# RashmikaDushan/MocapV2

Hardware: AMD Instinct MI355X
Metric: frames/sec (6-cam 1080p) (higher is better)
Workload: dtype u8+int64+f64; 1 GPU; 6-camera 1920x1080 synthetic IR frames, 8 markers (BASELINE.json configs[1]); cameras=6, width=1920, height=1080, markers=8, distortion=mild, frames_resident_in_hbm=True, batches_in_flight=3, resident_batches=3, status_ok=True, input=gray frames, parallelism=single launch, time-major

## Files before the change

include/mocap_hip.h:

```cpp
#ifndef MOCAP_HIP_H
#define MOCAP_HIP_H

#include <stddef.h>
#include <stdint.h>

#ifdef __cplusplus
extern "C" {
#endif

#define MOCAP_ABI_VERSION 7
#define MOCAP_API __attribute__((visibility("default")))

enum {
    MOCAP_OK = 0,
    MOCAP_E_INVALID = -1,
    MOCAP_E_HIP = -2,
    MOCAP_E_UNSUPPORTED = -3,
    MOCAP_E_STATE = -4
};

enum {
    MOCAP_BLOB_E_CANDIDATES = -2,
    MOCAP_BLOB_E_CONTOURS = -3,
    MOCAP_BLOB_E_STEPS = -4,
// ... 128 lines not shown
MOCAP_API int mocap_intrinsics_linearize(mocap_ctx_t ctx, int n_cams, const int32_t* view_offset_host,
                                         const int32_t* point_offset_host, const double* obj_xy_dev, const double* img_uv_dev,
                                         const double* kd_dev, const double* view_poses_dev, double lambda, double* cost_dev,
                                         double* gradient_dev, double* S_dev, double* rhs_dev, int32_t* status_dev, void* stream);

#define MOCAP_COMM_ID_BYTES 128
MOCAP_API int mocap_comm_unique_id(void* id_out );
MOCAP_API int mocap_comm_available(void);
MOCAP_API int mocap_comm_init(mocap_ctx_t ctx, const void* id , int rank, int world);
MOCAP_API int mocap_comm_share(mocap_ctx_t dst, mocap_ctx_t src);
MOCAP_API int mocap_comm_destroy(mocap_ctx_t ctx);
MOCAP_API int mocap_allgather_centroids(mocap_ctx_t ctx, const int32_t* local_records_dev, int32_t* gathered_dev,
                                        long ints_per_rank, void* stream);

MOCAP_API int mocap_tile_stats(mocap_ctx_t ctx, uint64_t* tiles, uint64_t* skipped);
MOCAP_API int mocap_profile_enable(mocap_ctx_t ctx, int on);
MOCAP_API int mocap_profile_read(mocap_ctx_t ctx, double ms[5], int launches[5]);

#ifdef __cplusplus
}
#endif
#endif
```

mocapv2_amd/_abi.py:

```python
import ctypes as C
import os

_HERE = os.path.dirname(os.path.abspath(__file__))
LIB_PATH = os.path.join(_HERE, "libmocap_hip.so")
ABI_VERSION = 7
COMM_ID_BYTES = 128


class MocapError(RuntimeError):
    def __init__(self, code, msg):
        super().__init__(f"libmocap_hip error {code}: {msg}")
        self.code = code


class BlobParams(C.Structure):
    _fields_ = [("ksize", C.c_int32), ("median", C.c_int32), ("thresh", C.c_double), ("min_area", C.c_double),
                ("min_circ", C.c_double)]


class UndistortInfo(C.Structure):
    _fields_ = [("identity", C.c_int32), ("compact_table", C.c_int32), ("early_out_provable", C.c_int32),
                ("max_source_weight", C.c_int32), ("sparse_path", C.c_int32)]


# ... 33 lines not shown
    "mocap_ba_residuals": [_vp, _dp, _i, _vp, _vp, _i, _i, C.POINTER(C.c_float), _ip, _vp],
    "mocap_fundamental_ransac": [_vp, _i, _vp, _vp, _ip, _vp, _i, _d, _i, _vp, _vp, _vp, _vp, _vp, _vp],
    "mocap_rig_bundle_adjust": [_vp, _i, _i, _i, _vp, _vp, _vp, _vp, _vp, _i, _d, _d, _vp, _vp, _vp],
    "mocap_rig_linearize": [_vp, _i, _i, _i, _vp, _vp, _vp, _vp, _vp, _d, _vp, _vp, _vp, _vp, _vp, _vp],
    "mocap_intrinsics_calibrate": [_vp, _i, _ip, _ip, _vp, _vp, _ip, _i, _i, _d, _d, _vp, _vp, _vp, _vp, _vp, _vp],
    "mocap_intrinsics_linearize": [_vp, _i, _ip, _ip, _vp, _vp, _vp, _vp, _d, _vp, _vp, _vp, _vp, _vp, _vp],
    "mocap_triangulate_batch": [_vp, _vp, _vp, _i, _i, _i, _vp, _vp, _vp],
    "mocap_reproject_batch": [_vp, _vp, _vp, _vp, _i, _i, _i, _vp, _vp, _vp],
    "mocap_comm_unique_id": [_vp],
    "mocap_comm_available": [],
    "mocap_comm_init": [_vp, _vp, _i, _i],
    "mocap_comm_share": [_vp, _vp],
    "mocap_comm_destroy": [_vp],
    "mocap_allgather_centroids": [_vp, _vp, _vp, _l, _vp],
    "mocap_tile_stats": [_vp, C.POINTER(C.c_uint64), C.POINTER(C.c_uint64)],
    "mocap_profile_enable": [_vp, _i],
    "mocap_profile_read": [_vp, _dp, _ip],
}

_lib = None


def load():
    global _lib
    if _lib is not None:
        return _lib
    if not os.path.exists(LIB_PATH):
        raise RuntimeError(f"{LIB_PATH} is missing: build it with `make -C mocapv2_amd/csrc` "
                           "(hipcc --offload-arch=gfx950); there is no CPU fallback")
    try:
# ... 19 lines not shown
```

mocapv2_amd/csrc/abi.hip:

```cpp
#include <hip/hip_runtime.h>
#include <stdint.h>
#include <stdio.h>
#include <stdarg.h>
#include <stdlib.h>
#include <string.h>
#include <math.h>
#include <string>
#include <vector>
#include <mutex>
#include <memory>
#include <dlfcn.h>
#include "../../include/mocap_hip.h"
#include "kernels.h"

using namespace mocap;

static_assert(sizeof(mocap_contour) == sizeof(ContourRec), "debug record layout");

static thread_local std::string g_err;

static int fail(int code, const char* fmt, ...)
{
    char buf[512];
    va_list ap;
// ... 54 lines not shown
        (void)hipSetDevice(device);
        if (last) { if (have_last) (void)hipEventSynchronize(last); (void)hipEventDestroy(last); }
        if (comm && destroy_comm) (void)destroy_comm(comm);
    }
};

struct Tuning {
    int rows = 68;
    int general_filter = 0;
    int skip_dark = 1;
    int dense_boxes = 0;
    int remap_pipeline = 1;
    int cluster = 1;
    int wide_quads_remap = 34, wide_quads_identity = 34;
    int wide_bands = 1;
    int wide_fork = 0;
    int box_prio = 0, scan_prio = 0, contour_prio = 0, corr_prio = 0;
    int box_stage_bytes = BOX_SCAP;
    int box_blocks_per_cu = 0;
    int box_timing = 0, contour_timing = 0, follow_timing = 0;
    int scan_wide = 1;
    int rows_staged = 0;
    int wide_blocks_per_cu = 3;
    int rows_stage_dw = -1;
    int scan_serial = 1;
    int scan_hotmap = 1;
    int scan_blocks_per_cu = 0;
    int scan_slices = 1;
    int excess_base = -1;
    int base_sel = 1;
    int probe_debug = 0;
    int contour_boxes = 1;
    int contours_split = 1;
    int contour_defer = 1;
    int mark_blocks_per_cu = 0;
    int contour_blocks_per_cu = 0;
    int corr_threads = 256;
    int corr_step_groups = 0;
};
struct TuneName { const char* name; int Tuning::*field; int lo, hi; };
static const TuneName kTuneNames[] = {
    {"rows", &Tuning::rows, 16, 68}, {"general_filter", &Tuning::general_filter, 0, 1}, {"skip_dark", &Tuning::skip_dark, 0, 1},
    {"dense_boxes", &Tuning::dense_boxes, 0, 1}, {"remap_pipeline", &Tuning::remap_pipeline, 0, 1}, {"cluster", &Tuning::cluster, 0, 1},
    {"wide_quads_remap", &Tuning::wide_quads_remap, 0, 100000}, {"wide_quads_identity", &Tuning::wide_quads_identity, 0, 100000},
    {"wide_bands", &Tuning::wide_bands, 1, 4}, {"wide_fork", &Tuning::wide_fork, 0, 1},
    {"box_prio", &Tuning::box_prio, 0, 1}, {"scan_prio", &Tuning::scan_prio, 0, 3}, {"contour_prio", &Tuning::contour_prio, 0, 3},
    {"corr_prio", &Tuning::corr_prio, 0, 3}, {"box_stage_bytes", &Tuning::box_stage_bytes, 0, BOX_SCAP},
    {"box_blocks_per_cu", &Tuning::box_blocks_per_cu, 0, 32}, {"box_timing", &Tuning::box_timing, 0, 1},
    {"contour_timing", &Tuning::contour_timing, 0, 1}, {"follow_timing", &Tuning::follow_timing, 0, 2}, {"scan_wide", &Tuning::scan_wide, 0, 1}, {"scan_hotmap", &Tuning::scan_hotmap, 0, 2}, {"scan_serial", &Tuning::scan_serial, 0, 1}, {"rows_staged", &Tuning::rows_staged, 0, 1}, {"wide_blocks_per_cu", &Tuning::wide_blocks_per_cu, 1, 8}, {"rows_stage_dw", &Tuning::rows_stage_dw, -1, 1 << 20}, {"scan_blocks_per_cu", &Tuning::scan_blocks_per_cu, 0, 64}, {"scan_slices", &Tuning::scan_slices, 1, 64}, {"excess_base", &Tuning::excess_base, -1, 254},
    {"base_sel", &Tuning::base_sel, 0, 1}, {"probe_debug", &Tuning::probe_debug, 0, 1}, {"contour_boxes", &Tuning::contour_boxes, 0, 1},
    {"contours_split", &Tuning::contours_split, 0, 1}, {"contour_blocks_per_cu", &Tuning::contour_blocks_per_cu, 0, 16}, {"mark_blocks_per_cu", &Tuning::mark_blocks_per_cu, 0, 16}, {"contour_defer", &Tuning::contour_defer, 0, 2}, {"corr_threads", &Tuning::corr_threads, 64, 256},
    {"corr_step_groups", &Tuning::corr_step_groups, 0, 0x7fffffff},
};
static bool tune_set(Tuning& t, const char* name, int v)
{
    for (const TuneName& n : kTuneNames)
        if (!strcmp(n.name, name)) {
            t.*(n.field) = v < n.lo ? n.lo : (v > n.hi ? n.hi : v);
            return true;
        }
// ... 377 lines not shown
    if (c->cells && c->last_images > 0) {
        HIP_TRY(hipDeviceSynchronize());
        Tiling t = tiling(c);
        size_t per = cells_per_image(c), n = per * (size_t)c->last_images;
        std::vector<uint32_t> w(n);
        HIP_TRY(hipMemcpy(w.data(), c->cells, sizeof(uint32_t) * n, hipMemcpyDeviceToHost));
        int valid_chunks = (c->H + t.rows - 1) / t.rows;
        total = (uint64_t)c->last_images * valid_chunks * t.n_strips;
        for (size_t i = 0; i < n; i++) full += w[i] >> 31;
    }
    if (tiles) *tiles = total;
    if (skipped) *skipped = total - full;
    return MOCAP_OK;
}

static int check_frames(mocap_ctx* c, const void* frames, int n_images, int cam_mod, int slot_base, size_t image_stride, int pitch)
{
    if (!c || !frames) return fail(MOCAP_E_INVALID, "null argument");
    if (n_images < 1) return fail(MOCAP_E_INVALID, "n_images = %d", n_images);
    if (cam_mod < 1 || slot_base < 0 || slot_base + cam_mod > c->n_slots)
        return fail(MOCAP_E_INVALID, "slots %d..%d not in 0..%d", slot_base, slot_base + cam_mod - 1, c->n_slots - 1);
    if (pitch < c->W) return fail(MOCAP_E_INVALID, "pitch %d < width %d", pitch, c->W);
    if (n_images > 1 && image_stride < (size_t)pitch * (c->H - 1) + c->W) return fail(MOCAP_E_INVALID, "image_stride too small");
    for (int s = slot_base; s < slot_base + cam_mod; s++)
        if (c->slot_state[s] == 0) return fail(MOCAP_E_STATE, "mocap_set_undistort was not called for slot %d", s);
    return 0;
}


static int excess_base(int thr_mul, int sel)
// ... 154 lines not shown
    a.srcbox = c->srcbox ? c->srcbox + (size_t)bt.slot_base * source_cells(c) : nullptr;
    a.remap_bits = p.remap_bits;
    a.cam_mod = bt.cam_mod; a.n_images = bt.n_images; a.n_steps = (bt.n_images + bt.cam_mod - 1) / bt.cam_mod;
    a.thr_mul = sb.thr_mul;
    a.rows_per_chunk = tl.rows; a.n_strips = tl.n_strips; a.n_chunks = tl.n_cgroups * 4;
    const size_t tr_words = c->mask_images * cells_per_image(c) * 4;
    a.tile_rows = c->tile_rows + (c->tile_rows_flip ? tr_words : 0);
    a.tile_rows_next = c->tile_rows + (c->tile_rows_flip ? 0 : tr_words);
    a.n_clear = c->tile_rows_hold[c->tile_rows_flip ^ 1];
    a.cluster = c->tune.cluster;
    a.cur_box = bt.own_mask ? c->cur_box : c->cur_box_ext;
    a.items = c->items; a.n_items = c->n_items; a.cap_items = (uint32_t)c->items.n;
    a.dense = sb.allow < 0;
    a.wide_tiles = c->wide_tiles; a.cap_wide = (uint32_t)c->wide_tiles.n; a.wide_quads_remap = c->tune.wide_quads_remap; a.wide_quads_identity = c->tune.wide_quads_identity;
    a.wide_bands = c->tune.wide_bands;
    if (c->W < 4 || p.direct) a.wide_tiles = nullptr;
    a.bayer = p.direct ? p.bl : BayerArgs{};
    a.stage_bytes = c->tune.box_stage_bytes;
    a.prio = c->tune.box_prio;
    a.ext_mask = bt.own_mask ? 0 : 1;
    return a;
}

static BrightArgs bright_args(const mocap_ctx* c, const Batch& bt, const FilterPath& p, const ScanBounds& sb, uint32_t* tile_rows, bool scan_zeroes)
{
    const Tiling tl = tiling(c);
    uint64_t ncx64 = (uint64_t)((c->W + 7) / 8);
    const uint64_t ncells = ncx64 * (uint64_t)((c->H + 7) / 8);
    int wide = (c->W % 16 == 0) && (bt.pitch % 16 == 0) && (bt.image_stride % 16 == 0) && (((uintptr_t)p.frames & 15) == 0) && ncx64 >= 4;
    if (wide && ncells * (ncx64 / 2) >= (1ull << 32)) wide = 0;
// ... 79 lines not shown

static int report_box_timing(mocap_ctx* c, const uint64_t* timing, hipStream_t s)
{
    std::vector<uint64_t> t((size_t)6 * c->box_grid);
    HIP_TRY(hipStreamSynchronize(s));
    HIP_TRY(hipMemcpy(t.data(), timing, sizeof(uint64_t) * t.size(), hipMemcpyDeviceToHost));
    double sum[6] = {0, 0, 0, 0, 0, 0}, mx = 0;
    for (int b = 0; b < c->box_grid; b++) {
        double tot = 0;
        for (int i = 0; i < 6; i++) { sum[i] += (double)t[6 * b + i]; if (i < 5) tot += (double)t[6 * b + i]; }
        mx = tot > mx ? tot : mx;
    }
    const double n = sum[5] > 0 ? sum[5] : 1;
    uint32_t cnt[16];
    HIP_TRY(hipMemcpy(cnt, c->n_items, sizeof(cnt), hipMemcpyDeviceToHost));
    fprintf(stderr, "[box] list: %u items, %u wide-tile entries\n", cnt[0], cnt[8]);
    fprintf(stderr, "[box] items %.0f (%.1f per wave) | cycles per item: header+wait %.0f, stage %.0f, patch %.0f, threshold %.0f, majority+next %.0f | busiest wave %.0f cycles\n",
            sum[5], sum[5] / c->box_grid, sum[0] / n, sum[1] / n, sum[2] / n, sum[3] / n, sum[4] / n, mx);
    return 0;
}

static int filter_boxes(mocap_ctx* c, const Batch& bt, const FilterPath& p, BoxArgs& a)
{
    const hipStream_t s = bt.s;
    Buf<uint64_t> timing;
    if (c->tune.box_timing) {
        TRY(timing.reserve((size_t)6 * c->box_grid));
        HIP_TRY(hipMemsetAsync(timing, 0, sizeof(uint64_t) * 6 * c->box_grid, s));
    }
    a.timing = timing;
    EvPair ev; bool on;
// ... 166 lines not shown
    EvPair p; bool on;
    prof_begin(c, 1, s, p, on);
    launch_contours(a, s);
    prof_end(c, 1, s, p, on);
    HIP_TRY(hipGetLastError());
    if (follow_dbg) TRY(report_follow_timing(follow_dbg, a.follow_grid, s));
    if (timing) TRY(report_contour_timing(timing, n_images, s));
    return 0;
}

static int grow_mask_group(mocap_ctx* c, size_t n_images)
{
    const size_t tiles = n_images * cells_per_image(c);
    TRY(c->mask.reserve(n_images * mask_image_words(c->H, c->wpr), true));
    TRY(c->cells.reserve(tiles, true));
    std::vector<uint32_t> init(tiles * 4);
    for (size_t i = 0; i < init.size(); i += 2) { init[i] = 0xffffffffu; init[i + 1] = 0u; }
    TRY(c->tile_rows.reserve(2 * init.size()));
    HIP_TRY(hipMemcpy(c->tile_rows, init.data(), sizeof(uint32_t) * init.size(), hipMemcpyHostToDevice));
    HIP_TRY(hipMemcpy(c->tile_rows + init.size(), init.data(), sizeof(uint32_t) * init.size(), hipMemcpyHostToDevice));
    const int hw0 = hot_map_words(c->H, c->W, 0), hw1 = hot_map_words(c->H, c->W, 1);
    TRY(c->hotmap.reserve(n_images * (hw0 > hw1 ? hw0 : hw1), true));
    for (size_t i = 0; i < init.size(); i++) init[i] = 1u;
    TRY(c->cur_box.reserve(init.size()));
    HIP_TRY(hipMemcpy(c->cur_box, init.data(), sizeof(uint32_t) * init.size(), hipMemcpyHostToDevice));
    const size_t cap = tiles * BOX_MAX_PARTS;
    if (cap > 0xffffffffull) return fail(MOCAP_E_UNSUPPORTED, "batch too large for the work list");
    TRY(c->items.reserve(cap));
    return c->wide_tiles.reserve(4 * tiles);
}
static int ensure_mask(mocap_ctx* c, int n_images)
{
// ... 602 lines not shown
```

mocapv2_amd/csrc/blob_boxes.hip:

```cpp
#include <hip/hip_runtime.h>
#include <stdint.h>
#include <type_traits>
#include "kernels.h"
#include "bayer.h"

namespace mocap {

namespace {

__device__ __forceinline__ uint32_t from_prev(uint32_t v)
{
    return (uint32_t)__builtin_amdgcn_update_dpp(0, (int)v, 0x138 , 0xf, 0xf, true);
}
__device__ __forceinline__ uint32_t from_next(uint32_t v)
{
    return (uint32_t)__builtin_amdgcn_update_dpp(0, (int)v, 0x130 , 0xf, 0xf, true);
}
__device__ __forceinline__ uint32_t dot4(uint32_t a, uint32_t sel, uint32_t acc) { return __builtin_amdgcn_udot4(a, sel, acc, false); }
__device__ __forceinline__ int uni(int v) { return __builtin_amdgcn_readfirstlane(v); }
__device__ __forceinline__ int imin(int a, int b) { return a < b ? a : b; }
__device__ __forceinline__ int imax(int a, int b) { return a > b ? a : b; }
__device__ __forceinline__ int taps5(int v, int n)
{
    int lo = v - 2 < 0 ? 0 : v - 2, hi = v + 2 > n - 1 ? n - 1 : v + 2;
// ... 76 lines not shown
__device__ __forceinline__ void choose_split(int nb, int h, int& nx, int& ny)
{
    int best = 0x7fffffff;
    nx = 1; ny = 1;
    for (int cx = 1; cx <= 4; cx++) {
        const int pb = (nb + cx - 1) / cx, Q = 2 * pb + 2;
        if (Q > 64) continue;
        const int rpw = 64 / Q, mr = BOX_HCAP / Q - 8;
        if (mr < 1) continue;
        const int cy = (h + mr - 1) / mr;
        if (cx * cy > BOX_MAX_PARTS) continue;
        const int ph = (h + cy - 1) / cy;
        const int cost = cx * cy * ((ph + 8 + rpw - 1) / rpw + 8);
        if (cost < best) { best = cost; nx = cx; ny = cy; }
    }
}

__global__ __launch_bounds__(256) void settle_tiles_kernel(BoxArgs a)
{
    const int lane = threadIdx.x & 63;
    if (a.zero8 && blockIdx.x == 0 && threadIdx.x < 8) a.zero8[threadIdx.x] = 0u;
    const int tiles = a.n_chunks * a.n_strips;
    const int n_all = a.n_clear > a.n_images ? a.n_clear : a.n_images;
    const int steps_all = (n_all + a.cam_mod - 1) / a.cam_mod;
    const long long total = (long long)tiles * a.cam_mod * steps_all;
    const long long i = (long long)blockIdx.x * 256 + threadIdx.x;
    int image = 0, chunk = 0, strip = 0;
    bool valid = i < total;
    if (valid) {
        const int t = (int)(i % steps_all);
        const long long rest = i / steps_all;
        const int slot = (int)(rest % a.cam_mod), tile = (int)(rest / a.cam_mod);
        image = t * a.cam_mod + slot;
        chunk = tile / a.n_strips; strip = tile - chunk * a.n_strips;
        valid = chunk * a.rows_per_chunk < a.H;
    }
    const size_t idx = ((size_t)image * a.n_chunks + chunk) * a.n_strips + strip;
    if (valid && !a.dense && image < n_all) {
        const uint4 nxt = *(const uint4*)(a.tile_rows_next + 4 * idx);
        if (nxt.x <= nxt.y) *(uint4*)(a.tile_rows_next + 4 * idx) = make_uint4(0xffffffffu, 0u, 0xffffffffu, 0u);
    }
    valid = valid && image < a.n_images;
    const int tile_r0 = chunk * a.rows_per_chunk, tile_r1 = imin(tile_r0 + a.rows_per_chunk, a.H) - 1;
    const int tile_x0 = 240 * strip, tile_x1 = imin(tile_x0 + 239, a.W - 1);
    int bx0 = 0, bx1 = a.W - 1, by0 = 0, by1 = a.H - 1;
    bool marked = valid;
    uint4 raw = make_uint4(0xffffffffu, 0u, 0xffffffffu, 0u);
    if (valid && !a.dense) {
        raw = *(const uint4*)(a.tile_rows + 4 * idx);
        marked = raw.x <= raw.y;
        if (marked) { by0 = (int)raw.x; by1 = (int)raw.y; bx0 = (int)raw.z; bx1 = (int)raw.w; }
    }
    int ox0 = imax(bx0, tile_x0) & ~7, ox1 = imin(imin(bx1, tile_x1) | 7, tile_x1);
    int oy0 = imax(by0, tile_r0), oy1 = imin(by1, tile_r1);
    if (marked && (ox0 > ox1 || oy0 > oy1)) marked = false;
    if (!marked) { ox0 = 1; ox1 = 0; oy0 = 1; oy1 = 0; }
    int nx = 0, ny = 0, nb = 0, h = 0;
    bool wide = false;
    int ix0 = ox0, ix1 = ox1, iy0 = oy0, iy1 = oy1;
    int ux0 = bx0, ux1 = bx1, uy0 = by0, uy1 = by1;
    bool emits = marked;
    if (marked && !a.dense && a.cluster) {
        const int c0 = chunk & ~1, s0 = strip & ~1;
        int n_marked = 0, first = -1, X0 = 0x7fffffff, X1 = -1, Y0 = 0x7fffffff, Y1 = -1;
        for (int k = 0; k < 4; k++) {
            const int cy = c0 + (k >> 1), sx = s0 + (k & 1);
            if (cy >= a.n_chunks || sx >= a.n_strips || cy * a.rows_per_chunk >= a.H) continue;
            const uint4 o = *(const uint4*)(a.tile_rows + 4 * (((size_t)image * a.n_chunks + cy) * a.n_strips + sx));
            if (o.x > o.y) continue;
            if (first < 0) first = k;
            n_marked++;
            Y0 = imin(Y0, (int)o.x); Y1 = imax(Y1, (int)o.y); X0 = imin(X0, (int)o.z); X1 = imax(X1, (int)o.w);
        }
        if (n_marked >= 2) {
            const int bx_lo = 240 * s0, bx_hi = imin(240 * (s0 + 2) - 1, a.W - 1), by_lo = c0 * a.rows_per_chunk, by_hi = imin((c0 + 2) * a.rows_per_chunk, a.H) - 1;
            const int ex0 = imax(X0, bx_lo) & ~7, ex1 = imin(X1 | 7, bx_hi), ey0 = imax(Y0, by_lo), ey1 = imin(Y1, by_hi);
            if (((ex1 - ex0 + 8) >> 3) <= 13 && ey1 - ey0 + 1 <= 100) {
                emits = first == ((chunk - c0) * 2 + (strip - s0));
                ix0 = ex0; ix1 = ex1; iy0 = ey0; iy1 = ey1;
                ux0 = X0; ux1 = X1; uy0 = Y0; uy1 = Y1;
            }
        }
    }
    if (marked) {
        nb = (ix1 - ix0 + 8) >> 3; h = iy1 - iy0 + 1;
        choose_split(nb, h, nx, ny);
        const int slot_ = image % a.cam_mod;
        const int limit = ((a.remap_bits >> slot_) & 1ull) ? a.wide_quads_remap : a.wide_quads_identity;
        wide = emits && ix0 == ox0 && ix1 == ox1 && iy0 == oy0 && iy1 == oy1 && a.wide_tiles != nullptr && 2 * nb + 2 * nx >= limit;
        if (wide) { ox0 = tile_x0; ox1 = tile_x1; ix0 = ox0; ix1 = ox1; }
    }
    const uint32_t nout_x = (uint32_t)ox0 | ((uint32_t)ox1 << 16), nout_y = (uint32_t)oy0 | ((uint32_t)oy1 << 16);

    bool need_clear = false;
    uint32_t pout_x = 1u, pout_y = 1u;
    if (valid) {
        uint4* cb = (uint4*)(a.cur_box + 4 * idx);
        if (!a.ext_mask) {
            const uint4 prev = *cb;
            pout_x = prev.x; pout_y = prev.y;
            const int px0 = (int)(prev.x & 0xffffu), px1 = (int)(prev.x >> 16), py0 = (int)(prev.y & 0xffffu), py1 = (int)(prev.y >> 16);
            if (px0 <= px1) need_clear = !(marked && ox0 <= px0 && px1 <= ox1 && oy0 <= py0 && py1 <= oy1);
            if (prev.x != nout_x || prev.y != nout_y || marked)
                *cb = make_uint4(nout_x, nout_y, (uint32_t)bx0 | ((uint32_t)bx1 << 16), (uint32_t)by0 | ((uint32_t)by1 << 16));
            if (a.cells[idx] != 0u) a.cells[idx] = 0u;
        } else {
            *cb = make_uint4(nout_x, nout_y, (uint32_t)bx0 | ((uint32_t)bx1 << 16), (uint32_t)by0 | ((uint32_t)by1 << 16));
            a.cells[idx] = 0u;
        }
    }
    for (uint64_t todo = __ballot(need_clear); todo; todo &= todo - 1) {
        const int src = __ffsll((long long)todo) - 1;
        const uint32_t cx = (uint32_t)__builtin_amdgcn_readlane((int)pout_x, src), cy = (uint32_t)__builtin_amdgcn_readlane((int)pout_y, src);
        const int cimage = __builtin_amdgcn_readlane(image, src);
        const int x0 = (int)(cx & 0xffffu), x1 = (int)(cx >> 16), y0 = (int)(cy & 0xffffu), y1 = (int)(cy >> 16);
        uint8_t* m = (uint8_t*)(a.mask + (size_t)cimage * mask_image_words(a.H, a.words_per_row));
        const int b0 = x0 >> 3, nr = y1 - y0 + 1, n = nr * ((x1 >> 3) - b0 + 1);
// ... 6 lines not shown
    if (uint64_t wb = __ballot(wide)) {
        const int nbands = a.wide_bands;
        uint32_t base_w = 0;
        if (lane == 0) base_w = atomicAdd(a.n_items + 8, (uint32_t)(__popcll(wb) * nbands));
        base_w = (uint32_t)__builtin_amdgcn_readfirstlane((int)base_w);
        const uint32_t ow = base_w + (uint32_t)(__popcll(wb & ((1ull << lane) - 1ull)) * nbands);
        if (wide) {
            const int hb = (oy1 - oy0 + nbands) / nbands;
            for (int b = 0; b < nbands; b++) {
                const int y0 = oy0 + b * hb, y1 = imin(y0 + hb - 1, oy1);
                if (ow + b < a.cap_wide)
                    a.wide_tiles[ow + b] = make_uint4((uint32_t)image, (uint32_t)(chunk * a.n_strips + strip), (uint32_t)y0, (uint32_t)(y0 <= y1 ? y1 : y0 - 1));
            }
        }
    }
    const int cnt = (wide || !emits) ? 0 : nx * ny;
    int incl = cnt;
#pragma unroll
    for (int d = 1; d < 64; d <<= 1) {
        const int o = __shfl_up(incl, d);
        if (lane >= d) incl += o;
    }
    const int wave_total = __builtin_amdgcn_readlane(incl, 63);
    if (wave_total == 0) return;
    uint32_t base = 0;
    if (lane == 0) base = atomicAdd(a.n_items, (uint32_t)wave_total);
    base = (uint32_t)__builtin_amdgcn_readfirstlane((int)base);
    uint32_t o = base + (uint32_t)(incl - cnt);
    if (cnt) {
        const int pb = (nb + nx - 1) / nx, ph = (h + ny - 1) / ny;
        for (int jy = 0; jy < ny; jy++)
            for (int jx = 0; jx < nx; jx++, o++) {
                const int x0 = ix0 + 8 * pb * jx, x1 = imin(x0 + 8 * pb - 1, ix1);
                const int y0 = iy0 + ph * jy, y1 = imin(y0 + ph - 1, iy1);
                if (o >= a.cap_items) continue;
                uint4 it;
                it.x = (uint32_t)image;
                it.y = (uint32_t)(chunk * a.n_strips + strip);
                it.z = (uint32_t)x0 | ((uint32_t)x1 << 16);
                it.w = (uint32_t)y0 | ((uint32_t)y1 << 16);
                if (x0 > x1 || y0 > y1) it.z = 1u;
                ((uint4*)a.items)[2 * o] = it;
                ((uint4*)a.items)[2 * o + 1] = make_uint4((uint32_t)ux0 | ((uint32_t)ux1 << 16), (uint32_t)uy0 | ((uint32_t)uy1 << 16), 0u, 0u);
            }
// ... 537 lines not shown
```

mocapv2_amd/csrc/blob_filter.hip:

```cpp
#include <hip/hip_runtime.h>
#include <stdint.h>
#include <type_traits>
#include "kernels.h"
#include "scan_mark.h"

namespace mocap {

__device__ __forceinline__ uint32_t lane_from_prev(uint32_t v)
{
    return (uint32_t)__builtin_amdgcn_update_dpp(0, (int)v, 0x138 , 0xf, 0xf, true);
}
__device__ __forceinline__ uint32_t lane_from_next(uint32_t v)
{
    return (uint32_t)__builtin_amdgcn_update_dpp(0, (int)v, 0x130 , 0xf, 0xf, true);
}
__device__ __forceinline__ uint32_t dot4(uint32_t a, uint32_t sel, uint32_t acc)
{
    return __builtin_amdgcn_udot4(a, sel, acc, false);
}

__device__ __forceinline__ uint32_t load_u32(const uint8_t* p)
{
    uint32_t v;
    __builtin_memcpy(&v, p, 4);
// ... 172 lines not shown
            const int c = 8 * cx, cc = c < a.W - 8 ? c : a.W - 8;
            sh[u] = (uint32_t)(8 * (c - cc));
#pragma unroll
            for (int j = 0; j < 8; j++) {
                int r = 8 * cr[u] + j;
                r = r < a.H ? r : a.H - 1;
                __builtin_memcpy(&v[u][j], img + ((uint32_t)r * (uint32_t)a.pitch + (uint32_t)cc), 8);
            }
        }
    }
    const int slot = image % a.cam_mod;
    const uint2* __restrict__ reach = a.reach + (size_t)slot * n;
    const uint8_t* __restrict__ cflags = a.cflags + (size_t)slot * n;
    uint32_t* __restrict__ rows = a.tile_rows + (size_t)image * a.n_chunks * a.n_strips * 4;
    const uint32_t base4 = (uint32_t)a.base * 0x01010101u, c8 = 8u * (uint32_t)a.base;
    uint32_t level[2] = {0u, 0u};
#pragma unroll
    for (int u = 0; u < 2; u++) {
        uint32_t acc = 0;
#pragma unroll
        for (int j = 0; j < 8; j++) {
            if (WIDE) {
                const uint32_t e2 = excess2_row(v[u][j].x, v[u][j].y, base4, c8);
                if (FULL || 8 * cr[u] + j < a.H) acc += e2;
            } else {
                uint64_t vv = (((uint64_t)v[u][j].y << 32) | v[u][j].x) >> sh[u];
                const uint32_t e2 = excess2_row((uint32_t)vv, (uint32_t)(vv >> 32), base4, c8);
                if (8 * cr[u] + j < a.H) acc += e2;
            }
        }
        if (MAP) level[u] = in_range[u] ? hot_level(a, acc) : 0u;
        else mark_hot_cell(a, reach, cflags, rows, ci[u], acc);
        if (a.probe && (image & 15) == 0) {
            const uint32_t alt4 = (uint32_t)a.base_alt * 0x01010101u, alt8 = 8u * (uint32_t)a.base_alt;
            uint32_t acc2 = 0;
#pragma unroll
            for (int j = 0; j < 8; j++) {
                const uint64_t vv = WIDE ? (((uint64_t)v[u][j].y << 32) | v[u][j].x) : ((((uint64_t)v[u][j].y << 32) | v[u][j].x) >> sh[u]);
                const uint32_t e2 = excess2_row((uint32_t)vv, (uint32_t)(vv >> 32), alt4, alt8);
                if (FULL || 8 * cr[u] + j < a.H) acc2 += e2;
            }
            const int n_cur = __popcll(__ballot((int)acc > a.hot)), n_alt = __popcll(__ballot((int)acc2 > a.hot_alt));
            if ((threadIdx.x & 63) == 0) {
                atomicAdd(&a.probe[PROBE_STRIDE * (bx & 127)], (uint32_t)n_cur);
                atomicAdd(&a.probe[PROBE_STRIDE * (bx & 127) + 1], (uint32_t)n_alt);
            }
        }
    }
    if (MAP) {
        const int lane = threadIdx.x & 63;
        uint32_t* __restrict__ hm = a.hotmap + (size_t)image * a.hot_words;
        if (WIDE) {
            uint32_t w = (level[0] | (level[1] << 2)) << (4 * (lane & 7));
            w |= (uint32_t)__builtin_amdgcn_update_dpp(0, (int)w, 0xB1 , 0xf, 0xf, true);
            w |= (uint32_t)__builtin_amdgcn_update_dpp(0, (int)w, 0x4E , 0xf, 0xf, true);
            w |= (uint32_t)__builtin_amdgcn_update_dpp(0, (int)w, 0x141 , 0xf, 0xf, true);
            if ((lane & 7) == 0 && w != 0u) hm[(bx * 256 + (int)threadIdx.x) >> 3] = w;
        } else {
#pragma unroll
            for (int u = 0; u < 2; u++) {
                uint32_t w = level[u] << (2 * (lane & 15));
                w |= (uint32_t)__builtin_amdgcn_update_dpp(0, (int)w, 0xB1, 0xf, 0xf, true);
// ... 15 lines not shown
    const int n_cells = ((a.W + 7) >> 3) * ((a.H + 7) >> 3);
    for (long long piece = (long long)blockIdx.x * 4 + wv; piece < (long long)wpi * a.n_images; piece += (long long)gridDim.x * 4) {
    const int image = (int)(piece / wpi), wave_word0 = (int)(piece - (long long)image * wpi) * 256;
    uint32_t* __restrict__ hm = a.hotmap + (size_t)image * a.hot_words;
    uint32_t wk[4];
#pragma unroll
    for (int k = 0; k < 4; k++) {
        const int wi = wave_word0 + 64 * k + lane;
        wk[k] = wi < a.hot_words ? hm[wi] : 0u;
    }
    if (__ballot((wk[0] | wk[1] | wk[2] | wk[3]) != 0u) == 0ull) continue;
#pragma unroll
    for (int k = 0; k < 4; k++)
        if (wk[k] != 0u) hm[wave_word0 + 64 * k + lane] = 0u;
    uint32_t (*tab)[5] = s_tab[wv];
    if (lane < 32) { tab[lane][0] = 0xffffffffu; tab[lane][1] = 0xffffffffu; tab[lane][2] = 0u; tab[lane][3] = 0xffffffffu; tab[lane][4] = 0u; }
    const int slot = image % a.cam_mod;
    const uint2* __restrict__ reach = a.reach + (size_t)slot * n_cells;
    const uint8_t* __restrict__ cflags = a.cflags + (size_t)slot * n_cells;
    uint32_t* __restrict__ rows = a.tile_rows + (size_t)image * a.n_chunks * a.n_strips * 4;
    auto widen = [&](int t, uint32_t ya, uint32_t yb, uint32_t xa, uint32_t xb) __attribute__((always_inline)) {
        const uint4 cur = *(const uint4*)(rows + 4 * t);
        if (cur.x <= ya && cur.y >= yb && cur.z <= xa && cur.w >= xb) return;
        atomicMin(&rows[4 * t], ya);
        atomicMax(&rows[4 * t + 1], yb);
        atomicMin(&rows[4 * t + 2], xa);
        atomicMax(&rows[4 * t + 3], xb);
    };
#pragma unroll 1
    for (int k = 0; k < 4; k++) {
        const uint32_t w = k == 0 ? wk[0] : (k == 1 ? wk[1] : (k == 2 ? wk[2] : wk[3]));
        const uint32_t nz = (w | (w >> 1)) & 0x55555555u;
        const int cnt = __popc(nz);
        if (__ballot(cnt != 0) == 0ull) continue;
        const int word0 = wave_word0 + 64 * k;
        int incl = cnt;
#pragma unroll
        for (int d = 1; d < 64; d <<= 1) {
            const int o = __shfl_up(incl, d);
            if (lane >= d) incl += o;
        }
        const int total = __builtin_amdgcn_readlane(incl, 63);
// ... 8 lines not shown
            const int e = e0 + lane;
            if (e < total) {
                const uint32_t v = s_list[wv][e];
                const int ci = 16 * (word0 + (int)(v >> 6)) + (int)((v >> 2) & 15u);
                if (ci < n_cells) {
                    const uint2 rc = reach[ci];
                    const int x0 = (int)(rc.x & 0xffffu), x1 = (int)(rc.x >> 16), y0 = (int)(rc.y & 0xffffu), y1 = (int)(rc.y >> 16);
                    if (x0 <= x1 && level_is_hot(v & 3u, cflags[ci])) {
                        const int xa = x0 - 4 > 0 ? x0 - 4 : 0, xb = x1 + 4 < a.W - 1 ? x1 + 4 : a.W - 1;
                        const int ya = y0 - 4 > 0 ? y0 - 4 : 0, yb = y1 + 4 < a.H - 1 ? y1 + 4 : a.H - 1;
                        const int ch0 = (int)(((uint32_t)ya * a.rows_magic) >> 23), ch1 = (int)(((uint32_t)yb * a.rows_magic) >> 23);
                        const int st0 = (int)(((uint32_t)xa * 34953u) >> 23), st1 = (int)(((uint32_t)xb * 34953u) >> 23);
                        for (int ch = ch0; ch <= ch1; ch++)
                            for (int st = st0; st <= st1; st++) {
                                const int t = ch * a.n_strips + st, q = t & 31;
                                const uint32_t old = atomicCAS(&tab[q][0], 0xffffffffu, (uint32_t)t);
                                if (old == 0xffffffffu || old == (uint32_t)t) {
                                    atomicMin(&tab[q][1], (uint32_t)ya); atomicMax(&tab[q][2], (uint32_t)yb);
                                    atomicMin(&tab[q][3], (uint32_t)xa); atomicMax(&tab[q][4], (uint32_t)xb);
                                } else
                                    widen(t, (uint32_t)ya, (uint32_t)yb, (uint32_t)xa, (uint32_t)xb);
                            }
                    }
                }
            }
        }
        __builtin_amdgcn_s_waitcnt(0xc07f);
        __builtin_amdgcn_wave_barrier();
    }
    if (lane < 32 && tab[lane][0] != 0xffffffffu) widen((int)tab[lane][0], tab[lane][1], tab[lane][2], tab[lane][3], tab[lane][4]);
    __builtin_amdgcn_s_waitcnt(0xc07f);
    __builtin_amdgcn_wave_barrier();
    }
}

template <bool WIDE, bool FULL = false, bool MAP = true>
__global__ __launch_bounds__(256) void bright_cells_kernel(BrightArgs a)
{
    if (a.prio == 1) __builtin_amdgcn_s_setprio(1);
    else if (a.prio == 2) __builtin_amdgcn_s_setprio(2);
    else if (a.prio == 3) __builtin_amdgcn_s_setprio(3);
    const uint32_t total = (uint32_t)a.blocks_x * (uint32_t)a.slice_images;
    if (a.zero_counters && blockIdx.x == 0) a.zero_counters[threadIdx.x] = 0u;
    if (a.block_ctr == nullptr) {
        for (uint32_t vb = blockIdx.x; vb < total; vb += gridDim.x) {
// ... 1003 lines not shown
```

mocapv2_amd/csrc/kernels.h:

```cpp
#pragma once
#include <hip/hip_runtime.h>
#include <stdint.h>

namespace mocap {

__host__ __device__ __forceinline__ uint32_t mask_word_index(int y, int k, int wpr)
{
    return ((uint32_t)(y >> 5) * (uint32_t)wpr + (uint32_t)k) * 32u + (uint32_t)(y & 31);
}
__host__ __device__ __forceinline__ uint32_t mask_byte_index(int y, int b, int wpr)
{
    return mask_word_index(y, b >> 2, wpr) * 4u + (uint32_t)(b & 3);
}
__host__ __device__ __forceinline__ size_t mask_image_words(int H, int wpr) { return (size_t)((H + 31) >> 5) * 32 * (size_t)wpr; }

__device__ __forceinline__ double wave_sum(double v)
{
#pragma unroll
    for (int o = 32; o > 0; o >>= 1) v += __shfl_down(v, o, 64);
    return v;
}
__device__ __forceinline__ double block_sum(double v, double* s_part )
{
    v = wave_sum(v);
// ... 71 lines not shown
    uint64_t remap_bits;
    int cam_mod, n_images, n_steps;
    int thr_mul;
    int rows_per_chunk, n_strips, n_chunks;
    uint32_t* tile_rows;
    uint32_t* tile_rows_next;
    int n_clear;
    int cluster;
    uint32_t* cur_box;
    BoxItem* items; uint32_t* n_items; uint32_t cap_items;
    uint64_t* timing;
    int prio;
    int stage_bytes;
    uint4* wide_tiles;
    uint32_t cap_wide; int wide_quads_remap, wide_quads_identity, wide_bands;
    uint32_t* zero8;
    int dense;
    int ext_mask;
    BayerArgs bayer;
};
void launch_settle_tiles(const BoxArgs& a, hipStream_t s);
void launch_box_filter(const BoxArgs& a, int grid, hipStream_t s, bool bayer = false);
int box_filter_blocks_per_cu();
void launch_srcbox(const uint32_t* map4, ushort4* srcbox, int H, int W, hipStream_t s);

struct MapArgs {
    double K[9], dist[5];
    int H, W;
    uint32_t* map;
    uint32_t* mapw;
// ... 296 lines not shown
```

mocapv2_amd/csrc/scan_mark.h:

```cpp
#pragma once
#include <hip/hip_runtime.h>
#include <stdint.h>
#include "kernels.h"

namespace mocap {

__device__ __forceinline__ uint32_t excess2_row(uint32_t lo, uint32_t hi, uint32_t base4, uint32_t c8)
{
    uint32_t s = __builtin_amdgcn_sad_u8(lo, base4, 0u);
    s = __builtin_amdgcn_sad_u8(lo, 0u, s);
    s = __builtin_amdgcn_sad_u8(hi, base4, s);
    s = __builtin_amdgcn_sad_u8(hi, 0u, s);
    return s - c8;
}

__device__ __forceinline__ void widen_tile_boxes(const BrightArgs& a, const uint2 rc, uint32_t* __restrict__ rows)
{
    const int x0 = (int)(rc.x & 0xffffu), x1 = (int)(rc.x >> 16), y0 = (int)(rc.y & 0xffffu), y1 = (int)(rc.y >> 16);
    if (x0 > x1) return;
    const int xa = x0 - 4 > 0 ? x0 - 4 : 0, xb = x1 + 4 < a.W - 1 ? x1 + 4 : a.W - 1;
    const int ya = y0 - 4 > 0 ? y0 - 4 : 0, yb = y1 + 4 < a.H - 1 ? y1 + 4 : a.H - 1;
    const int ch0 = (int)(((uint32_t)ya * a.rows_magic) >> 23), ch1 = (int)(((uint32_t)yb * a.rows_magic) >> 23);
    const int st0 = (int)(((uint32_t)xa * 34953u) >> 23), st1 = (int)(((uint32_t)xb * 34953u) >> 23);
    for (int ch = ch0; ch <= ch1; ch++)
        for (int st = st0; st <= st1; st++) {
            const int t = ch * a.n_strips + st;
            const uint4 cur = *(const uint4*)(rows + 4 * t);
            if (cur.x <= (uint32_t)ya && cur.y >= (uint32_t)yb && cur.z <= (uint32_t)xa && cur.w >= (uint32_t)xb) continue;
            atomicMin(&rows[4 * t], (uint32_t)ya);
            atomicMax(&rows[4 * t + 1], (uint32_t)yb);
            atomicMin(&rows[4 * t + 2], (uint32_t)xa);
            atomicMax(&rows[4 * t + 3], (uint32_t)xb);
        }
}

__device__ __forceinline__ void mark_hot_cell(const BrightArgs& a, const uint2* __restrict__ reach, const uint8_t* __restrict__ cflags,
                                              uint32_t* __restrict__ rows, int ci, uint32_t acc)
{
    if ((int)acc > a.hot_corner) {
        const uint2 rc = reach[ci];
        const uint32_t fl = cflags[ci];
        if ((int)acc > ((fl & 2u) ? a.hot_corner : (fl & 1u) ? a.hot_edge : a.hot)) widen_tile_boxes(a, rc, rows);
    }
}

__device__ __forceinline__ uint32_t hot_level(const BrightArgs& a, uint32_t acc)
{
// ... 9 lines not shown
```

mocapv2_amd/engine.py:

```python
import ctypes as C
import threading

import numpy as np
import torch

from . import _abi

MAX_BLOBS = 128
GRAY_SHIFT = 15
REC_INTS = 2 + 2 * MAX_BLOBS


def _ptr(t):
    return C.c_void_p(t.data_ptr()) if t is not None else None


def _stream():
    return C.c_void_p(torch.cuda.current_stream().cuda_stream)


def _dbl(a, n):
    a = np.ascontiguousarray(a, np.float64).reshape(-1)
    assert a.size == n, (a.size, n)
    return a, a.ctypes.data_as(C.POINTER(C.c_double))
# ... 457 lines not shown

    def allgather_centroids(self, local, out=None):
        assert local.is_cuda and local.is_contiguous() and local.dtype == torch.int32
        world = self.comm_world
        if out is None:
            out = torch.empty((world * local.shape[0],) + tuple(local.shape[1:]), dtype=torch.int32, device=local.device)
        assert out.is_contiguous() and out.numel() == world * local.numel() and out.dtype == torch.int32
        _abi.check(self.lib.mocap_allgather_centroids(self._h, _ptr(local), _ptr(out), local.numel(), _stream()))
        return out

    def tile_stats(self):
        a, b = C.c_uint64(0), C.c_uint64(0)
        _abi.check(self.lib.mocap_tile_stats(self._h, C.byref(a), C.byref(b)))
        return a.value, b.value

    def profile(self, on=True):
        _abi.check(self.lib.mocap_profile_enable(self._h, int(on)))

    def profile_read(self):
        ms = (C.c_double * 5)()
        n = (C.c_int * 5)()
        _abi.check(self.lib.mocap_profile_read(self._h, ms, n))
        return {"filter_ms": ms[0], "filter_launches": n[0], "contour_ms": ms[1], "contour_launches": n[1],
                "corr_ms": ms[2], "corr_launches": n[2], "scan_ms": ms[3], "scan_launches": n[3],
                "settle_ms": ms[4], "settle_launches": n[4]}


class BAProblem:

    def __init__(self, ctx, pts, valid=None):
# ... 50 lines not shown
```

Baseline: 374,700 frames/s.

## Track tile column coverage as bitmask and optionally split wide tiles into runs

Each tile's x-extent is now stored as a 32-bit occupancy mask of 8-pixel column groups, updated with atomicOr, replacing the atomicMin/atomicMax pair. The settle kernel derives bounds from the mask. Under a new wide_split tuning flag it can emit separate work items per contiguous column run instead of routing the tile to the wide-tile path. The aim is fewer atomics per mark and less wasted box work on sparse wide tiles. The split path is off by default, and the added mask decoding costs some extra ALU work.

```diff
diff --git a/include/mocap_hip.h b/include/mocap_hip.h
--- a/include/mocap_hip.h
+++ b/include/mocap_hip.h
@@ -166,6 +166,7 @@
                                         long ints_per_rank, void* stream);
 
 MOCAP_API int mocap_tile_stats(mocap_ctx_t ctx, uint64_t* tiles, uint64_t* skipped);
+MOCAP_API int mocap_work_stats(mocap_ctx_t ctx, uint64_t* items, uint64_t* wide_entries, uint64_t* split_tiles);
 MOCAP_API int mocap_profile_enable(mocap_ctx_t ctx, int on);
 MOCAP_API int mocap_profile_read(mocap_ctx_t ctx, double ms[5], int launches[5]);
 
diff --git a/mocapv2_amd/_abi.py b/mocapv2_amd/_abi.py
--- a/mocapv2_amd/_abi.py
+++ b/mocapv2_amd/_abi.py
@@ -71,6 +71,7 @@
     "mocap_comm_destroy": [_vp],
     "mocap_allgather_centroids": [_vp, _vp, _vp, _l, _vp],
     "mocap_tile_stats": [_vp, C.POINTER(C.c_uint64), C.POINTER(C.c_uint64)],
+    "mocap_work_stats": [_vp, C.POINTER(C.c_uint64), C.POINTER(C.c_uint64), C.POINTER(C.c_uint64)],
     "mocap_profile_enable": [_vp, _i],
     "mocap_profile_read": [_vp, _dp, _ip],
 }
diff --git a/mocapv2_amd/csrc/abi.hip b/mocapv2_amd/csrc/abi.hip
--- a/mocapv2_amd/csrc/abi.hip
+++ b/mocapv2_amd/csrc/abi.hip
@@ -92,6 +92,7 @@
     int cluster = 1;
     int wide_quads_remap = 34, wide_quads_identity = 34;
     int wide_bands = 1;
+    int wide_split = 0;
     int wide_fork = 0;
     int box_prio = 0, scan_prio = 0, contour_prio = 0, corr_prio = 0;
     int box_stage_bytes = BOX_SCAP;
@@ -121,7 +122,7 @@
     {"rows", &Tuning::rows, 16, 68}, {"general_filter", &Tuning::general_filter, 0, 1}, {"skip_dark", &Tuning::skip_dark, 0, 1},
     {"dense_boxes", &Tuning::dense_boxes, 0, 1}, {"remap_pipeline", &Tuning::remap_pipeline, 0, 1}, {"cluster", &Tuning::cluster, 0, 1},
     {"wide_quads_remap", &Tuning::wide_quads_remap, 0, 100000}, {"wide_quads_identity", &Tuning::wide_quads_identity, 0, 100000},
-    {"wide_bands", &Tuning::wide_bands, 1, 4}, {"wide_fork", &Tuning::wide_fork, 0, 1},
+    {"wide_bands", &Tuning::wide_bands, 1, 4}, {"wide_split", &Tuning::wide_split, 0, 1}, {"wide_fork", &Tuning::wide_fork, 0, 1},
     {"box_prio", &Tuning::box_prio, 0, 1}, {"scan_prio", &Tuning::scan_prio, 0, 3}, {"contour_prio", &Tuning::contour_prio, 0, 3},
     {"corr_prio", &Tuning::corr_prio, 0, 3}, {"box_stage_bytes", &Tuning::box_stage_bytes, 0, BOX_SCAP},
     {"box_blocks_per_cu", &Tuning::box_blocks_per_cu, 0, 32}, {"box_timing", &Tuning::box_timing, 0, 1},
@@ -529,6 +530,21 @@
     return MOCAP_OK;
 }
 
+int mocap_work_stats(mocap_ctx_t c, uint64_t* items, uint64_t* wide_entries, uint64_t* split_tiles)
+{
+    if (!c) return fail(MOCAP_E_INVALID, "null context");
+    if (set_device(c)) return MOCAP_E_HIP;
+    uint32_t cnt[16] = {0};
+    if (c->n_items) {
+        HIP_TRY(hipDeviceSynchronize());
+        HIP_TRY(hipMemcpy(cnt, c->n_items, sizeof(cnt), hipMemcpyDeviceToHost));
+    }
+    if (items) *items = cnt[0];
+    if (wide_entries) *wide_entries = cnt[8];
+    if (split_tiles) *split_tiles = cnt[4];
+    return MOCAP_OK;
+}
+
 static int check_frames(mocap_ctx* c, const void* frames, int n_images, int cam_mod, int slot_base, size_t image_stride, int pitch)
 {
     if (!c || !frames) return fail(MOCAP_E_INVALID, "null argument");
@@ -713,6 +729,7 @@
     a.dense = sb.allow < 0;
     a.wide_tiles = c->wide_tiles; a.cap_wide = (uint32_t)c->wide_tiles.n; a.wide_quads_remap = c->tune.wide_quads_remap; a.wide_quads_identity = c->tune.wide_quads_identity;
     a.wide_bands = c->tune.wide_bands;
+    a.wide_split = c->tune.wide_split;
     if (c->W < 4 || p.direct) a.wide_tiles = nullptr;
     a.bayer = p.direct ? p.bl : BayerArgs{};
     a.stage_bytes = c->tune.box_stage_bytes;
@@ -822,7 +839,7 @@
     const double n = sum[5] > 0 ? sum[5] : 1;
     uint32_t cnt[16];
     HIP_TRY(hipMemcpy(cnt, c->n_items, sizeof(cnt), hipMemcpyDeviceToHost));
-    fprintf(stderr, "[box] list: %u items, %u wide-tile entries\n", cnt[0], cnt[8]);
+    fprintf(stderr, "[box] list: %u items, %u wide-tile entries, %u split tiles\n", cnt[0], cnt[8], cnt[4]);
     fprintf(stderr, "[box] items %.0f (%.1f per wave) | cycles per item: header+wait %.0f, stage %.0f, patch %.0f, threshold %.0f, majority+next %.0f | busiest wave %.0f cycles\n",
             sum[5], sum[5] / c->box_grid, sum[0] / n, sum[1] / n, sum[2] / n, sum[3] / n, sum[4] / n, mx);
     return 0;
@@ -1019,8 +1036,8 @@
     const size_t tiles = n_images * cells_per_image(c);
     TRY(c->mask.reserve(n_images * mask_image_words(c->H, c->wpr), true));
     TRY(c->cells.reserve(tiles, true));
-    std::vector<uint32_t> init(tiles * 4);
-    for (size_t i = 0; i < init.size(); i += 2) { init[i] = 0xffffffffu; init[i + 1] = 0u; }
+    std::vector<uint32_t> init(tiles * 4, 0u);
+    for (size_t i = 0; i < init.size(); i += 4) init[i] = 0xffffffffu;
     TRY(c->tile_rows.reserve(2 * init.size()));
     HIP_TRY(hipMemcpy(c->tile_rows, init.data(), sizeof(uint32_t) * init.size(), hipMemcpyHostToDevice));
     HIP_TRY(hipMemcpy(c->tile_rows + init.size(), init.data(), sizeof(uint32_t) * init.size(), hipMemcpyHostToDevice));
diff --git a/mocapv2_amd/csrc/blob_boxes.hip b/mocapv2_amd/csrc/blob_boxes.hip
--- a/mocapv2_amd/csrc/blob_boxes.hip
+++ b/mocapv2_amd/csrc/blob_boxes.hip
@@ -114,6 +114,15 @@
         const int cost = cx * cy * ((ph + 8 + rpw - 1) / rpw + 8);
         if (cost < best) { best = cost; nx = cx; ny = cy; }
     }
+}
+
+__device__ __forceinline__ int cols_first(uint32_t cols, int strip) { return imax(240 * strip - 8 + 8 * (__ffs((int)cols) - 1), 0); }
+__device__ __forceinline__ int cols_last(uint32_t cols, int strip, int W) { return imin(240 * strip - 8 + 8 * (31 - __clz((int)cols)) + 7, W - 1); }
+__device__ __forceinline__ void first_run(uint32_t m, int& s, int& n)
+{
+    s = __ffs((int)m) - 1;
+    const uint32_t inv = ~(m >> s);
+    n = inv ? __ffs((int)inv) - 1 : 32 - s;
 }
 
 __global__ __launch_bounds__(256) void settle_tiles_kernel(BoxArgs a)
@@ -138,28 +147,29 @@
     const size_t idx = ((size_t)image * a.n_chunks + chunk) * a.n_strips + strip;
     if (valid && !a.dense && image < n_all) {
         const uint4 nxt = *(const uint4*)(a.tile_rows_next + 4 * idx);
-        if (nxt.x <= nxt.y) *(uint4*)(a.tile_rows_next + 4 * idx) = make_uint4(0xffffffffu, 0u, 0xffffffffu, 0u);
+        if (nxt.x <= nxt.y) *(uint4*)(a.tile_rows_next + 4 * idx) = make_uint4(0xffffffffu, 0u, 0u, 0u);
     }
     valid = valid && image < a.n_images;
     const int tile_r0 = chunk * a.rows_per_chunk, tile_r1 = imin(tile_r0 + a.rows_per_chunk, a.H) - 1;
     const int tile_x0 = 240 * strip, tile_x1 = imin(tile_x0 + 239, a.W - 1);
     int bx0 = 0, bx1 = a.W - 1, by0 = 0, by1 = a.H - 1;
     bool marked = valid;
-    uint4 raw = make_uint4(0xffffffffu, 0u, 0xffffffffu, 0u);
+    uint32_t cols = 0u;
     if (valid && !a.dense) {
-        raw = *(const uint4*)(a.tile_rows + 4 * idx);
-        marked = raw.x <= raw.y;
-        if (marked) { by0 = (int)raw.x; by1 = (int)raw.y; bx0 = (int)raw.z; bx1 = (int)raw.w; }
+        const uint4 raw = *(const uint4*)(a.tile_rows + 4 * idx);
+        marked = raw.x <= raw.y && raw.z != 0u;
+        if (marked) { cols = raw.z; by0 = (int)raw.x; by1 = (int)raw.y; bx0 = cols_first(cols, strip); bx1 = cols_last(cols, strip, a.W); }
     }
     int ox0 = imax(bx0, tile_x0) & ~7, ox1 = imin(imin(bx1, tile_x1) | 7, tile_x1);
     int oy0 = imax(by0, tile_r0), oy1 = imin(by1, tile_r1);
     if (marked && (ox0 > ox1 || oy0 > oy1)) marked = false;
     if (!marked) { ox0 = 1; ox1 = 0; oy0 = 1; oy1 = 0; }
     int nx = 0, ny = 0, nb = 0, h = 0;
-    bool wide = false;
+    bool wide = false, split = false;
+    int split_parts = 0;
     int ix0 = ox0, ix1 = ox1, iy0 = oy0, iy1 = oy1;
     int ux0 = bx0, ux1 = bx1, uy0 = by0, uy1 = by1;
-    bool emits = marked;
+    bool emits = marked, clustered = false;
     if (marked && !a.dense && a.cluster) {
         const int c0 = chunk & ~1, s0 = strip & ~1;
         int n_marked = 0, first = -1, X0 = 0x7fffffff, X1 = -1, Y0 = 0x7fffffff, Y1 = -1;
@@ -167,15 +177,16 @@
             const int cy = c0 + (k >> 1), sx = s0 + (k & 1);
             if (cy >= a.n_chunks || sx >= a.n_strips || cy * a.rows_per_chunk >= a.H) continue;
             const uint4 o = *(const uint4*)(a.tile_rows + 4 * (((size_t)image * a.n_chunks + cy) * a.n_strips + sx));
-            if (o.x > o.y) continue;
+            if (o.x > o.y || o.z == 0u) continue;
             if (first < 0) first = k;
             n_marked++;
-            Y0 = imin(Y0, (int)o.x); Y1 = imax(Y1, (int)o.y); X0 = imin(X0, (int)o.z); X1 = imax(X1, (int)o.w);
+            Y0 = imin(Y0, (int)o.x); Y1 = imax(Y1, (int)o.y); X0 = imin(X0, cols_first(o.z, sx)); X1 = imax(X1, cols_last(o.z, sx, a.W));
         }
         if (n_marked >= 2) {
             const int bx_lo = 240 * s0, bx_hi = imin(240 * (s0 + 2) - 1, a.W - 1), by_lo = c0 * a.rows_per_chunk, by_hi = imin((c0 + 2) * a.rows_per_chunk, a.H) - 1;
             const int ex0 = imax(X0, bx_lo) & ~7, ex1 = imin(X1 | 7, bx_hi), ey0 = imax(Y0, by_lo), ey1 = imin(Y1, by_hi);
             if (((ex1 - ex0 + 8) >> 3) <= 13 && ey1 - ey0 + 1 <= 100) {
+                clustered = true;
                 emits = first == ((chunk - c0) * 2 + (strip - s0));
                 ix0 = ex0; ix1 = ex1; iy0 = ey0; iy1 = ey1;
                 ux0 = X0; ux1 = X1; uy0 = Y0; uy1 = Y1;
@@ -187,7 +198,20 @@
         choose_split(nb, h, nx, ny);
         const int slot_ = image % a.cam_mod;
         const int limit = ((a.remap_bits >> slot_) & 1ull) ? a.wide_quads_remap : a.wide_quads_identity;
-        wide = emits && ix0 == ox0 && ix1 == ox1 && iy0 == oy0 && iy1 == oy1 && a.wide_tiles != nullptr && 2 * nb + 2 * nx >= limit;
+        wide = emits && ix0 == ox0 && ix1 == ox1 && iy0 == oy0 && iy1 == oy1 && 2 * nb + 2 * nx >= limit;
+        if (wide && a.wide_split && !clustered && !a.dense) {
+            int parts = 0, nruns = 0;
+            for (uint32_t m = (cols >> 1) & 0x3fffffffu; m && parts <= BOX_MAX_PARTS;) {
+                int rs, rn, rx, ry;
+                first_run(m, rs, rn);
+                m &= ~(((1u << rn) - 1u) << rs);
+                choose_split(rn, h, rx, ry);
+                parts = 2 * rn + 2 * rx >= limit ? BOX_MAX_PARTS + 1 : parts + rx * ry;
+                nruns++;
+            }
+            if (nruns >= 2 && parts <= BOX_MAX_PARTS) { split = true; split_parts = parts; }
+        }
+        wide = wide && !split && a.wide_tiles != nullptr;
         if (wide) { ox0 = tile_x0; ox1 = tile_x1; ix0 = ox0; ix1 = ox1; }
     }
     const uint32_t nout_x = (uint32_t)ox0 | ((uint32_t)ox1 << 16), nout_y = (uint32_t)oy0 | ((uint32_t)oy1 << 16);
@@ -200,7 +224,7 @@
             const uint4 prev = *cb;
             pout_x = prev.x; pout_y = prev.y;
             const int px0 = (int)(prev.x & 0xffffu), px1 = (int)(prev.x >> 16), py0 = (int)(prev.y & 0xffffu), py1 = (int)(prev.y >> 16);
-            if (px0 <= px1) need_clear = !(marked && ox0 <= px0 && px1 <= ox1 && oy0 <= py0 && py1 <= oy1);
+            if (px0 <= px1) need_clear = !(marked && !split && ox0 <= px0 && px1 <= ox1 && oy0 <= py0 && py1 <= oy1);
             if (prev.x != nout_x || prev.y != nout_y || marked)
                 *cb = make_uint4(nout_x, nout_y, (uint32_t)bx0 | ((uint32_t)bx1 << 16), (uint32_t)by0 | ((uint32_t)by1 << 16));
             if (a.cells[idx] != 0u) a.cells[idx] = 0u;
@@ -237,7 +261,9 @@
             }
         }
     }
-    const int cnt = (wide || !emits) ? 0 : nx * ny;
+    if (const uint64_t sb = __ballot(split))
+        if (lane == 0) atomicAdd(a.n_items + 4, (uint32_t)__popcll(sb));
+    const int cnt = (wide || !emits) ? 0 : (split ? split_parts : nx * ny);
     int incl = cnt;
 #pragma unroll
     for (int d = 1; d < 64; d <<= 1) {
@@ -250,7 +276,20 @@
     if (lane == 0) base = atomicAdd(a.n_items, (uint32_t)wave_total);
     base = (uint32_t)__builtin_amdgcn_readfirstlane((int)base);
     uint32_t o = base + (uint32_t)(incl - cnt);
-    if (cnt) {
+    if (!cnt) return;
+    uint32_t runs = split ? (cols >> 1) & 0x3fffffffu : 1u;
+    while (runs) {
+        if (split) {
+            int rs, rn;
+            first_run(runs, rs, rn);
+            runs &= ~(((1u << rn) - 1u) << rs);
+            nb = rn;
+            choose_split(nb, h, nx, ny);
+            ix0 = tile_x0 + 8 * rs; ix1 = imin(ix0 + 8 * rn - 1, tile_x1);
+            ux0 = imax(ix0 - ((rs == 0 && (cols & 1u)) ? 8 : 0), 0);
+            ux1 = imin(ix1 + ((rs + rn == 30 && (cols >> 31)) ? 8 : 0), a.W - 1);
+        } else
+            runs = 0u;
         const int pb = (nb + nx - 1) / nx, ph = (h + ny - 1) / ny;
         for (int jy = 0; jy < ny; jy++)
             for (int jx = 0; jx < nx; jx++, o++) {
diff --git a/mocapv2_amd/csrc/blob_filter.hip b/mocapv2_amd/csrc/blob_filter.hip
--- a/mocapv2_amd/csrc/blob_filter.hip
+++ b/mocapv2_amd/csrc/blob_filter.hip
@@ -210,7 +210,7 @@
     const uint8_t* __restrict__ cflags = a.cflags + (size_t)slot * n;
     uint32_t* __restrict__ rows = a.tile_rows + (size_t)image * a.n_chunks * a.n_strips * 4;
     const uint32_t base4 = (uint32_t)a.base * 0x01010101u, c8 = 8u * (uint32_t)a.base;
-    uint32_t level[2] = {0u, 0u};
+    uint32_t level[2] = {0u, 0u}, sums[2] = {0u, 0u};
 #pragma unroll
     for (int u = 0; u < 2; u++) {
         uint32_t acc = 0;
@@ -226,7 +226,7 @@
             }
         }
         if (MAP) level[u] = in_range[u] ? hot_level(a, acc) : 0u;
-        else mark_hot_cell(a, reach, cflags, rows, ci[u], acc);
+        else sums[u] = acc;
         if (a.probe && (image & 15) == 0) {
             const uint32_t alt4 = (uint32_t)a.base_alt * 0x01010101u, alt8 = 8u * (uint32_t)a.base_alt;
             uint32_t acc2 = 0;
@@ -242,6 +242,10 @@
                 atomicAdd(&a.probe[PROBE_STRIDE * (bx & 127) + 1], (uint32_t)n_alt);
             }
         }
+    }
+    if (!MAP) {
+#pragma unroll
+        for (int u = 0; u < 2; u++) mark_hot_cell(a, reach, cflags, rows, ci[u], sums[u]);
     }
     if (MAP) {
         const int lane = threadIdx.x & 63;
@@ -287,18 +291,17 @@
     for (int k = 0; k < 4; k++)
         if (wk[k] != 0u) hm[wave_word0 + 64 * k + lane] = 0u;
     uint32_t (*tab)[5] = s_tab[wv];
-    if (lane < 32) { tab[lane][0] = 0xffffffffu; tab[lane][1] = 0xffffffffu; tab[lane][2] = 0u; tab[lane][3] = 0xffffffffu; tab[lane][4] = 0u; }
+    if (lane < 32) { tab[lane][0] = 0xffffffffu; tab[lane][1] = 0xffffffffu; tab[lane][2] = 0u; tab[lane][3] = 0u; }
     const int slot = image % a.cam_mod;
     const uint2* __restrict__ reach = a.reach + (size_t)slot * n_cells;
     const uint8_t* __restrict__ cflags = a.cflags + (size_t)slot * n_cells;
     uint32_t* __restrict__ rows = a.tile_rows + (size_t)image * a.n_chunks * a.n_strips * 4;
-    auto widen = [&](int t, uint32_t ya, uint32_t yb, uint32_t xa, uint32_t xb) __attribute__((always_inline)) {
+    auto widen = [&](int t, uint32_t ya, uint32_t yb, uint32_t bits) __attribute__((always_inline)) {
         const uint4 cur = *(const uint4*)(rows + 4 * t);
-        if (cur.x <= ya && cur.y >= yb && cur.z <= xa && cur.w >= xb) return;
+        if (cur.x <= ya && cur.y >= yb && (cur.z & bits) == bits) return;
         atomicMin(&rows[4 * t], ya);
         atomicMax(&rows[4 * t + 1], yb);
-        atomicMin(&rows[4 * t + 2], xa);
-        atomicMax(&rows[4 * t + 3], xb);
+        atomicOr(&rows[4 * t + 2], bits);
     };
 #pragma unroll 1
     for (int k = 0; k < 4; k++) {
@@ -337,12 +340,13 @@
                         for (int ch = ch0; ch <= ch1; ch++)
                             for (int st = st0; st <= st1; st++) {
                                 const int t = ch * a.n_strips + st, q = t & 31;
+                                const uint32_t bits = tile_col_bits(st, xa, xb);
                                 const uint32_t old = atomicCAS(&tab[q][0], 0xffffffffu, (uint32_t)t);
                                 if (old == 0xffffffffu || old == (uint32_t)t) {
                                     atomicMin(&tab[q][1], (uint32_t)ya); atomicMax(&tab[q][2], (uint32_t)yb);
-                                    atomicMin(&tab[q][3], (uint32_t)xa); atomicMax(&tab[q][4], (uint32_t)xb);
+                                    atomicOr(&tab[q][3], bits);
                                 } else
-                                    widen(t, (uint32_t)ya, (uint32_t)yb, (uint32_t)xa, (uint32_t)xb);
+                                    widen(t, (uint32_t)ya, (uint32_t)yb, bits);
                             }
                     }
                 }
@@ -351,7 +355,7 @@
         __builtin_amdgcn_s_waitcnt(0xc07f);
         __builtin_amdgcn_wave_barrier();
     }
-    if (lane < 32 && tab[lane][0] != 0xffffffffu) widen((int)tab[lane][0], tab[lane][1], tab[lane][2], tab[lane][3], tab[lane][4]);
+    if (lane < 32 && tab[lane][0] != 0xffffffffu) widen((int)tab[lane][0], tab[lane][1], tab[lane][2], tab[lane][3]);
     __builtin_amdgcn_s_waitcnt(0xc07f);
     __builtin_amdgcn_wave_barrier();
     }
diff --git a/mocapv2_amd/csrc/kernels.h b/mocapv2_amd/csrc/kernels.h
--- a/mocapv2_amd/csrc/kernels.h
+++ b/mocapv2_amd/csrc/kernels.h
@@ -109,6 +109,7 @@
     int stage_bytes;
     uint4* wide_tiles;
     uint32_t cap_wide; int wide_quads_remap, wide_quads_identity, wide_bands;
+    int wide_split;
     uint32_t* zero8;
     int dense;
     int ext_mask;
diff --git a/mocapv2_amd/csrc/scan_mark.h b/mocapv2_amd/csrc/scan_mark.h
--- a/mocapv2_amd/csrc/scan_mark.h
+++ b/mocapv2_amd/csrc/scan_mark.h
@@ -14,6 +14,12 @@
     return s - c8;
 }
 
+__device__ __forceinline__ uint32_t tile_col_bits(int st, int xa, int xb)
+{
+    const int g0 = (xa - 240 * st + 8) >> 3, g1 = (xb - 240 * st + 8) >> 3;
+    return (2u << (g1 < 31 ? g1 : 31)) - (1u << (g0 > 0 ? g0 : 0));
+}
+
 __device__ __forceinline__ void widen_tile_boxes(const BrightArgs& a, const uint2 rc, uint32_t* __restrict__ rows)
 {
     const int x0 = (int)(rc.x & 0xffffu), x1 = (int)(rc.x >> 16), y0 = (int)(rc.y & 0xffffu), y1 = (int)(rc.y >> 16);
@@ -25,12 +31,12 @@
     for (int ch = ch0; ch <= ch1; ch++)
         for (int st = st0; st <= st1; st++) {
             const int t = ch * a.n_strips + st;
+            const uint32_t bits = tile_col_bits(st, xa, xb);
             const uint4 cur = *(const uint4*)(rows + 4 * t);
-            if (cur.x <= (uint32_t)ya && cur.y >= (uint32_t)yb && cur.z <= (uint32_t)xa && cur.w >= (uint32_t)xb) continue;
+            if (cur.x <= (uint32_t)ya && cur.y >= (uint32_t)yb && (cur.z & bits) == bits) continue;
             atomicMin(&rows[4 * t], (uint32_t)ya);
             atomicMax(&rows[4 * t + 1], (uint32_t)yb);
-            atomicMin(&rows[4 * t + 2], (uint32_t)xa);
-            atomicMax(&rows[4 * t + 3], (uint32_t)xb);
+            atomicOr(&rows[4 * t + 2], bits);
         }
 }
 
diff --git a/mocapv2_amd/engine.py b/mocapv2_amd/engine.py
--- a/mocapv2_amd/engine.py
+++ b/mocapv2_amd/engine.py
@@ -495,6 +495,11 @@
         _abi.check(self.lib.mocap_tile_stats(self._h, C.byref(a), C.byref(b)))
         return a.value, b.value
 
+    def work_stats(self):
+        a, b, c = C.c_uint64(0), C.c_uint64(0), C.c_uint64(0)
+        _abi.check(self.lib.mocap_work_stats(self._h, C.byref(a), C.byref(b), C.byref(c)))
+        return a.value, b.value, c.value
+
     def profile(self, on=True):
         _abi.check(self.lib.mocap_profile_enable(self._h, int(on)))
 
```

Result: faster. 379,000 frames/s, median of 6 (+1.1%).
